# thedonutfactory/rs-tfhe

Hardware: AMD Instinct MI355X
Metric: gate-bootstraps/sec (hom_nand, SECURITY_128_BIT) (higher is better)
Workload: dtype f64

## Files before the change

rs-tfhe_amd/csrc/key_switch_mfma.hpp:

```cpp
#pragma once
#include <hip/hip_runtime.h>
#include <stdint.h>

#include <type_traits>

namespace tfhe {

constexpr int kKmWaves = 4;
constexpr int kKmFrags = 1;
constexpr int kKmRows = 32 * kKmFrags * kKmWaves;
constexpr int kKmSlots = 4;
constexpr int kKmAhead = kKmSlots - 1;
constexpr int kKmAbBytes = 32 * kKmFrags * 16 * 4;
constexpr int kKmAbQ = kKmAbBytes / 256;
constexpr int kKmColBlocks = 2;
constexpr int kKmMaxTiles = 12 / kKmFrags;

__host__ __device__ constexpr int ks_mfma_tpw(int nt) { return (nt + kKmWaves - 1) / kKmWaves; }
__host__ __device__ constexpr int ks_mfma_slot_bytes(int nt) { return ks_mfma_tpw(nt) * kKmWaves * 1024; }
__host__ __device__ constexpr size_t ks_mfma_lds_bytes(int nt) {
  return (size_t)kKmSlots * ks_mfma_slot_bytes(nt) + (size_t)kKmWaves * 2 * kKmAbBytes + (size_t)kKmWaves * 256;
}
__host__ __device__ __forceinline__ int ks_mfma_total_tiles(int n) { return (n + 1 + 31) / 32; }
__host__ __device__ __forceinline__ int ks_mfma_tiles(int n) { return (ks_mfma_total_tiles(n) + kKmColBlocks - 1) / kKmColBlocks; }
__host__ __device__ __forceinline__ int ks_mfma_block_tiles(int n, int cb) {
  const int tiles = ks_mfma_total_tiles(n);
  return tiles / kKmColBlocks + (cb < tiles % kKmColBlocks ? 1 : 0);
}
__host__ __device__ __forceinline__ int ks_mfma_block_first(int n, int cb) {
  const int tiles = ks_mfma_total_tiles(n), base = tiles / kKmColBlocks, rem = tiles % kKmColBlocks;
  return cb * base + (cb < rem ? cb : rem);
}
__host__ __device__ __forceinline__ size_t ks_mfma_key_bytes(int n, int t) {
  return (size_t)4 * (64 * 2 * t) * ks_mfma_total_tiles(n) * 1024;
}
constexpr size_t kKmKeyTailPad = 64 * 1024;

__host__ __device__ __forceinline__ uint32_t ks_plane_byte(uint32_t w, int p) {
  uint32_t s = 0;
  for (int q = 0; q <= p; ++q) {
    s = w & 0xFFu;
    const uint32_t sext = (s & 0x80u) ? (s | 0xFFFFFF00u) : s;
    w = (w - sext) >> 8;
  }
  return s;
}

template <class Word>
__device__ __forceinline__ uint4 ks_plane_fragment(int p, Word word) {
  uint32_t o[4];
#pragma unroll
  for (int q = 0; q < 4; ++q) {
    uint32_t d = 0;
#pragma unroll
    for (int e = 0; e < 4; ++e) d |= ks_plane_byte(word(q, e), p) << (8 * e);
    o[q] = d;
  }
  return make_uint4(o[0], o[1], o[2], o[3]);
}

__global__ void k_ksk_planes(const uint32_t *__restrict__ eng, unsigned char *__restrict__ out, int n, int t,
                             size_t chunks) {
  const size_t idx = (size_t)blockIdx.x * blockDim.x + threadIdx.x;
  if (idx >= chunks) return;
  const int lane = (int)(idx & 63);
  size_t r = idx >> 6;
  const int S = 64 * 2 * t, tiles = ks_mfma_total_tiles(n);
  const size_t per_plane = (size_t)S * tiles;
  const int p = (int)(r / per_plane);
  r -= (size_t)p * per_plane;
  int cb = 0;
  while (cb + 1 < kKmColBlocks && r >= (size_t)S * ks_mfma_block_first(n, cb + 1)) ++cb;
  r -= (size_t)S * ks_mfma_block_first(n, cb);
  const int nt = ks_mfma_block_tiles(n, cb);
  const int s = (int)(r / (size_t)nt), c = (int)(r % (size_t)nt);
  const int col = (ks_mfma_block_first(n, cb) + c) * 32 + (lane & 31), kb = lane >> 5;
  const int blk = s / (2 * t), u = s % (2 * t), j = u >> 1, hh = u & 1;
  const int rw = (n + 1 + 3) & ~3;
  reinterpret_cast<uint4 *>(out)[idx] = ks_plane_fragment(p, [=](int cc, int k) {
    const int i = 16 * blk + 8 * hh + 4 * kb + cc;
    const size_t row = ((size_t)i * t + j) * 4 + k;
    return (col <= n && k != 0) ? eng[row * (size_t)rw + col] : 0u;
  });
}

using km_i32x4 = __attribute__((ext_vector_type(4))) int;
using km_i32x16 = __attribute__((ext_vector_type(16))) int;
using km_u32x4 = __attribute__((ext_vector_type(4))) unsigned int;

__device__ __forceinline__ void km_dma16(uint32_t voff, const void *sbase, uint32_t lds) {
  uint32_t keep;
  asm volatile(
      "s_mov_b32 %0, m0\n\t"
      "s_mov_b32 m0, %3\n\t"
      "s_nop 0\n\t"
      "global_load_lds_dwordx4 %1, %2\n\t"
      "s_mov_b32 m0, %0"
      : "=&s"(keep)
      : "v"(voff), "s"(sbase), "s"(lds)
      : "memory");
}
__device__ __forceinline__ void km_dma4(uint32_t voff, const void *sbase, uint32_t lds) {
  uint32_t keep;
  asm volatile(
      "s_mov_b32 %0, m0\n\t"
      "s_mov_b32 m0, %3\n\t"
      "s_nop 0\n\t"
      "global_load_lds_dword %1, %2\n\t"
      "s_mov_b32 m0, %0"
      : "=&s"(keep)
      : "v"(voff), "s"(sbase), "s"(lds)
      : "memory");
}

struct KmPos {
  int blk, u;
};

template <int NT>
__global__ __launch_bounds__(64 * kKmWaves, 2) void k_key_switch_mfma(const uint32_t *__restrict__ lv1,
                                                                       const unsigned char *__restrict__ ksk8,
                                                                       int n, int t, uint32_t *__restrict__ out,
                                                                       size_t count,
                                                                       unsigned long long *clk,
                                                                       int ksplit) {
  constexpr int N = 1024, D = kKmAhead, WAVES = kKmWaves, R = kKmFrags;
  constexpr int TPW = ks_mfma_tpw(NT), SLOT = ks_mfma_slot_bytes(NT), OPS = TPW + R;
  const unsigned long long clk0 = clk ? __builtin_amdgcn_s_memtime() : 0ull;
  const unsigned long long rtc0 = clk ? __builtin_amdgcn_s_memrealtime() : 0ull;
  extern __shared__ __attribute__((aligned(16))) unsigned char km_smem[];
  const int tid = threadIdx.x, lane = tid & 63;
  const int wave = __builtin_amdgcn_readfirstlane(tid >> 6);
  const uint32_t lds_base = (uint32_t)(size_t)(__attribute__((address_space(3))) unsigned char *)km_smem;
  const uint32_t off_ab = (uint32_t)(kKmSlots * SLOT) + (uint32_t)wave * 2u * kKmAbBytes;
  const uint32_t off_dump = (uint32_t)(kKmSlots * SLOT) + (uint32_t)(WAVES * 2 * kKmAbBytes) + (uint32_t)wave * 256u;
  const unsigned lin = blockIdx.x + gridDim.x * (blockIdx.y + gridDim.y * blockIdx.z);
  const unsigned combos = gridDim.y * gridDim.z, combo = lin % combos, rest = lin / combos;
  const int cb = (int)(combo % gridDim.y), plane = (int)(combo / gridDim.y);
  const unsigned n_rb = gridDim.x / (unsigned)ksplit;
  const int kchunk = (int)(rest / n_rb);
  const int blk0 = kchunk * (64 / ksplit);
  const size_t row0 = (size_t)(rest % n_rb) * kKmRows + (size_t)wave * (32 * R);
  const int nt_blk = ks_mfma_block_tiles(n, cb), tile0 = ks_mfma_block_first(n, cb);
  const bool full = nt_blk == NT;
  const int spb = 2 * t, S = 64 * spb;
  const uint32_t prec = 1u << (31 - 2 * t);
  const uint32_t v16 = (uint32_t)lane * 16u;
  const uint32_t v4 = (uint32_t)(((lane >> 4) * (N + 1) + (lane & 15)) * 4);
  const uint32_t *ab_row0 = lv1 + row0 * (size_t)(N + 1);

  const unsigned char *kplane = ksk8 + ((size_t)plane * ks_mfma_total_tiles(n) + (size_t)tile0) * S * 1024;
  uint32_t koff[TPW];
#pragma unroll
  for (int i = 0; i < TPW; ++i) {
    const int tile = wave + i * WAVES;
    koff[i] = (uint32_t)(tile < nt_blk ? tile : nt_blk - 1) * 1024u + v16;
  }
  const uint32_t kstride = (uint32_t)nt_blk * 1024u;
  const int steps = S / ksplit;
#pragma unroll
  for (int i = 0; i < TPW; ++i) koff[i] += (uint32_t)(blk0 * spb) * kstride;
  auto dma_key = [&](uint32_t slot) {
#pragma unroll
    for (int i = 0; i < TPW; ++i) {
      km_dma16(koff[i], kplane, slot + (uint32_t)(wave + i * WAVES) * 1024u);
      koff[i] += kstride;
    }
  };

  for (int q = 0; q < kKmAbQ; ++q) km_dma4(v4, ab_row0 + (size_t)(4 * q) * (N + 1) + 16 * blk0, lds_base + off_ab + (uint32_t)q * 256u);
  for (int d = 0; d < D; ++d) dma_key(lds_base + (uint32_t)d * SLOT);
  asm volatile("s_waitcnt vmcnt(0)" ::: "memory");
  __builtin_amdgcn_s_barrier();
  asm volatile("" ::: "memory");

  km_i32x16 acc[R][NT];
  const uint32_t a_lane = (uint32_t)((lane & 31) * 64 + (lane >> 5) * 16);
  auto read_a = [&](const KmPos &q, int f) -> km_u32x4 {
    const unsigned char *abuf = km_smem + off_ab + (uint32_t)(q.blk & 1) * kKmAbBytes + a_lane + (uint32_t)(q.u & 1) * 32u;
    return *reinterpret_cast<const km_u32x4 *>(abuf + f * (32 * 64));
  };
  auto build_a = [&](const KmPos &q, km_u32x4 w) -> km_i32x4 {
    const uint32_t sh = (uint32_t)(27 - 2 * (q.u >> 1));
    km_u32x4 a;
    a.x = 1u << (((w.x + prec) >> sh) & 0x18u);
    a.y = 1u << (((w.y + prec) >> sh) & 0x18u);
    a.z = 1u << (((w.z + prec) >> sh) & 0x18u);
    a.w = 1u << (((w.w + prec) >> sh) & 0x18u);
    return __builtin_bit_cast(km_i32x4, a);
  };
  auto make_a = [&](const KmPos &q, int f) -> km_i32x4 { return build_a(q, read_a(q, f)); };
  KmPos cur{blk0, 0};
  km_i32x4 A[R];
#pragma unroll
  for (int f = 0; f < R; ++f) A[f] = make_a(cur, f);
  constexpr int PRE = NT < 3 ? NT : 3;
  constexpr int H = NT / 2;
  km_i32x4 Bpre[PRE];
#pragma unroll
  for (int c = 0; c < PRE; ++c) Bpre[c] = *reinterpret_cast<const km_i32x4 *>(km_smem + v16 + c * 1024);
#pragma unroll
  for (int f = 0; f < R; ++f)
#pragma unroll
    for (int c = 0; c < NT; ++c) acc[f][c] = km_i32x16{0, 0, 0, 0, 0, 0, 0, 0, 0, 0, 0, 0, 0, 0, 0, 0};
  auto run = [&](auto full_c) {
    constexpr bool FULL = decltype(full_c)::value;
#pragma unroll 1
    for (int g = 0; g < steps; ++g) {
      const unsigned char *slot = km_smem + (uint32_t)(g % kKmSlots) * SLOT + v16;
      const unsigned char *slot_next = km_smem + (uint32_t)((g + 1) % kKmSlots) * SLOT + v16;
      km_i32x4 B[NT];
#pragma unroll
      for (int c = 0; c < PRE; ++c) B[c] = Bpre[c];
#pragma unroll
      for (int c = 0; c < H; ++c) {
        if (c + PRE < NT) B[c + PRE] = *reinterpret_cast<const km_i32x4 *>(slot + (c + PRE) * 1024);
#pragma unroll
        for (int f = 0; f < R; ++f) acc[f][c] = __builtin_amdgcn_mfma_i32_32x32x32_i8(A[f], B[c], acc[f][c], 0, 0, 0);
      }
      __builtin_amdgcn_sched_barrier(0);
      asm volatile("s_waitcnt vmcnt(%0)" ::"n"((D - 2) * OPS) : "memory");
      __builtin_amdgcn_s_barrier();
      asm volatile("" ::: "memory");
      const uint32_t dslot = lds_base + (uint32_t)((g + D) % kKmSlots) * SLOT;
      const int nblk = (cur.blk + 1) & 63;
      const uint32_t nbuf = lds_base + off_ab + (uint32_t)((cur.blk + 1) & 1) * kKmAbBytes;
      const int u_now = cur.u;
      constexpr int PIECES = TPW + R + 2;
      km_i32x4 A_next[R];
      km_u32x4 Aw[R];
      auto piece = [&](int it) {
        if (it == 0) {
          if (++cur.u == spb) {
            cur.u = 0;
            cur.blk = (cur.blk + 1) & 63;
          }
#pragma unroll
          for (int f = 0; f < R; ++f) Aw[f] = read_a(cur, f);
#pragma unroll
          for (int c = 0; c < PRE; ++c) Bpre[c] = *reinterpret_cast<const km_i32x4 *>(slot_next + c * 1024);
        } else if (it == PIECES - 2) {
#pragma unroll
          for (int f = 0; f < R; ++f) A_next[f] = build_a(cur, Aw[f]);
        } else {
          const int d = it - 1 - (it > PIECES - 2 ? 1 : 0);
          if (d < TPW) {
            km_dma16(koff[d], kplane, dslot + (uint32_t)(wave + d * WAVES) * 1024u);
            koff[d] += kstride;
          } else {
            const int q0 = R * u_now + (d - TPW);
            const uint32_t *s0 = ab_row0 + (size_t)(4 * (q0 & (kKmAbQ - 1))) * (N + 1) + 16 * nblk;
            km_dma4(v4, s0, q0 < kKmAbQ ? nbuf + (uint32_t)q0 * 256u : lds_base + off_dump);
          }
        }
      };
#pragma unroll
      for (int c = H; c < NT; ++c) {
        if (c + PRE < NT) B[c + PRE] = *reinterpret_cast<const km_i32x4 *>(slot + (c + PRE) * 1024);
        if (c < NT - 1 || FULL) {
#pragma unroll
          for (int f = 0; f < R; ++f) acc[f][c] = __builtin_amdgcn_mfma_i32_32x32x32_i8(A[f], B[c], acc[f][c], 0, 0, 0);
        }
        __builtin_amdgcn_sched_barrier(0);
        if (c - H < PIECES) piece(c - H);
        __builtin_amdgcn_sched_barrier(0);
      }
#pragma unroll
      for (int it = NT - H; it < PIECES; ++it) piece(it);
#pragma unroll
      for (int f = 0; f < R; ++f) A[f] = A_next[f];
    }
  };
  if (full)
    run(std::true_type{});
  else
    run(std::false_type{});
  {
    const int sh8 = 8 * plane;
    const int row_lim = (int)(count > row0 ? (count - row0 < 32 * R ? count - row0 : 32 * R) : 0) - 4 * (lane >> 5);
    const int col_lane = tile0 * 32 + (lane & 31);
    const uint32_t lane_off = (uint32_t)((4 * (lane >> 5)) * (n + 1) + col_lane) * 4u;
    unsigned char *obase = reinterpret_cast<unsigned char *>(out + row0 * (size_t)(n + 1));
    const uint32_t row_bytes = (uint32_t)(n + 1) * 4u;
#pragma unroll
    for (int f = 0; f < R; ++f)
#pragma unroll
      for (int c = 0; c < NT; ++c) {
        const bool col_ok = col_lane + 32 * c <= n && c < nt_blk;
        const bool is_body = col_lane + 32 * c == n && plane == 0 && kchunk == 0;
#pragma unroll
        for (int e = 0; e < 16; ++e) {
          const int er = 32 * f + (e & 3) + 8 * (e >> 2);
          if (col_ok && er < row_lim) {
            uint32_t v = 0u - ((uint32_t)acc[f][c][e] << sh8);
            if (is_body) v += lv1[(row0 + (size_t)(er + 4 * (lane >> 5))) * (size_t)(N + 1) + N];
            unsigned char *uni = obase + (size_t)((uint32_t)er * row_bytes + (uint32_t)(c * 128));
            if (v) atomicAdd(reinterpret_cast<uint32_t *>(uni + lane_off), v);
          }
        }
      }
  }
  asm volatile("s_waitcnt vmcnt(0)" ::: "memory");
  if (clk && tid == 0) {
    atomicAdd(&clk[0], __builtin_amdgcn_s_memtime() - clk0);
    atomicAdd(&clk[1], __builtin_amdgcn_s_memrealtime() - rtc0);
  }
}

}
```

Before: 197,900.

## Use sparse SMFMAC i8 instructions for key-switch one-hot digit matmul

```diff
diff --git a/rs-tfhe_amd/csrc/key_switch_mfma.hpp b/rs-tfhe_amd/csrc/key_switch_mfma.hpp
--- a/rs-tfhe_amd/csrc/key_switch_mfma.hpp
+++ b/rs-tfhe_amd/csrc/key_switch_mfma.hpp
@@ -73,20 +73,28 @@
   while (cb + 1 < kKmColBlocks && r >= (size_t)S * ks_mfma_block_first(n, cb + 1)) ++cb;
   r -= (size_t)S * ks_mfma_block_first(n, cb);
   const int nt = ks_mfma_block_tiles(n, cb);
-  const int s = (int)(r / (size_t)nt), c = (int)(r % (size_t)nt);
-  const int col = (ks_mfma_block_first(n, cb) + c) * 32 + (lane & 31), kb = lane >> 5;
-  const int blk = s / (2 * t), u = s % (2 * t), j = u >> 1, hh = u & 1;
+  const int s = (int)(r / (size_t)(2 * nt)), c = (int)(r % (size_t)(2 * nt)) >> 1, q = (int)(r & 1);
+  const int col = (ks_mfma_block_first(n, cb) + c) * 32 + (lane & 31), h = lane >> 5;
+  const int blk = s / t, j = s % t;
   const int rw = (n + 1 + 3) & ~3;
   reinterpret_cast<uint4 *>(out)[idx] = ks_plane_fragment(p, [=](int cc, int k) {
-    const int i = 16 * blk + 8 * hh + 4 * kb + cc;
+    const int i = 16 * blk + 8 * h + 4 * q + cc;
     const size_t row = ((size_t)i * t + j) * 4 + k;
     return (col <= n && k != 0) ? eng[row * (size_t)rw + col] : 0u;
   });
 }
 
 using km_i32x4 = __attribute__((ext_vector_type(4))) int;
+using km_i32x8 = __attribute__((ext_vector_type(8))) int;
 using km_i32x16 = __attribute__((ext_vector_type(16))) int;
 using km_u32x4 = __attribute__((ext_vector_type(4))) unsigned int;
+
+constexpr int kKmSparseA = 0x00010001;
+__device__ __forceinline__ uint32_t km_sparse_idx(km_u32x4 lo, km_u32x4 hi, uint32_t prec, uint32_t sh) {
+  auto dg = [&](uint32_t w) { return ((w + prec) >> sh) & 3u; };
+  return dg(lo.x) | (dg(lo.y) << 4) | (dg(lo.z) << 8) | (dg(lo.w) << 12) | (dg(hi.x) << 16) | (dg(hi.y) << 20) |
+         (dg(hi.z) << 24) | (dg(hi.w) << 28);
+}
 
 __device__ __forceinline__ void km_dma16(uint32_t voff, const void *sbase, uint32_t lds) {
   uint32_t keep;
@@ -149,104 +157,116 @@
   const uint32_t v4 = (uint32_t)(((lane >> 4) * (N + 1) + (lane & 15)) * 4);
   const uint32_t *ab_row0 = lv1 + row0 * (size_t)(N + 1);
 
-  const unsigned char *kplane = ksk8 + ((size_t)plane * ks_mfma_total_tiles(n) + (size_t)tile0) * S * 1024;
-  uint32_t koff[TPW];
-#pragma unroll
-  for (int i = 0; i < TPW; ++i) {
-    const int tile = wave + i * WAVES;
-    koff[i] = (uint32_t)(tile < nt_blk ? tile : nt_blk - 1) * 1024u + v16;
-  }
-  const uint32_t kstride = (uint32_t)nt_blk * 1024u;
+  constexpr int T0 = (NT + 1) / 2, T1 = NT - T0;
+  static_assert(kKmSlots == 4 && D == 3, "unit g + D is the other half of a K-step: the ring arithmetic below");
+  static_assert(2 * T0 <= TPW * WAVES, "a unit's pieces fit the slot");
+  const uint32_t kstride = (uint32_t)nt_blk * 2048u;
+  const unsigned char *kwalk = ksk8 + ((size_t)plane * ks_mfma_total_tiles(n) + (size_t)tile0) * S * 1024 +
+                                (size_t)(blk0 * t) * kstride;
+  uint32_t spoff[2][TPW];
+#pragma unroll
+  for (int hf = 0; hf < 2; ++hf) {
+    const int up = hf ? 2 * (nt_blk - T0) : 2 * T0;
+#pragma unroll
+    for (int i = 0; i < TPW; ++i) {
+      const int pc = wave + i * WAVES, last = up > 0 ? up - 1 : 0;
+      spoff[hf][i] = (uint32_t)(hf * T0 * 2048) + (uint32_t)(pc < last ? pc : last) * 1024u;
+    }
+  }
   const int steps = S / ksplit;
-#pragma unroll
-  for (int i = 0; i < TPW; ++i) koff[i] += (uint32_t)(blk0 * spb) * kstride;
-  auto dma_key = [&](uint32_t slot) {
-#pragma unroll
-    for (int i = 0; i < TPW; ++i) {
-      km_dma16(koff[i], kplane, slot + (uint32_t)(wave + i * WAVES) * 1024u);
-      koff[i] += kstride;
-    }
+  auto dma_key = [&](int ks, int half, uint32_t slot) {
+    const unsigned char *src = kwalk + (size_t)ks * kstride;
+#pragma unroll
+    for (int i = 0; i < TPW; ++i) km_dma16(v16, src + spoff[half][i], slot + (uint32_t)(wave + i * WAVES) * 1024u);
   };
 
   for (int q = 0; q < kKmAbQ; ++q) km_dma4(v4, ab_row0 + (size_t)(4 * q) * (N + 1) + 16 * blk0, lds_base + off_ab + (uint32_t)q * 256u);
-  for (int d = 0; d < D; ++d) dma_key(lds_base + (uint32_t)d * SLOT);
+#pragma unroll
+  for (int d = 0; d < D; ++d) dma_key(d >> 1, d & 1, lds_base + (uint32_t)d * SLOT);
   asm volatile("s_waitcnt vmcnt(0)" ::: "memory");
   __builtin_amdgcn_s_barrier();
   asm volatile("" ::: "memory");
 
   km_i32x16 acc[R][NT];
   const uint32_t a_lane = (uint32_t)((lane & 31) * 64 + (lane >> 5) * 16);
-  auto read_a = [&](const KmPos &q, int f) -> km_u32x4 {
-    const unsigned char *abuf = km_smem + off_ab + (uint32_t)(q.blk & 1) * kKmAbBytes + a_lane + (uint32_t)(q.u & 1) * 32u;
+  auto read_a = [&](const KmPos &q, int f, int hi) -> km_u32x4 {
+    const unsigned char *abuf = km_smem + off_ab + (uint32_t)(q.blk & 1) * kKmAbBytes + a_lane + (uint32_t)hi * 32u;
     return *reinterpret_cast<const km_u32x4 *>(abuf + f * (32 * 64));
   };
-  auto build_a = [&](const KmPos &q, km_u32x4 w) -> km_i32x4 {
-    const uint32_t sh = (uint32_t)(27 - 2 * (q.u >> 1));
-    km_u32x4 a;
-    a.x = 1u << (((w.x + prec) >> sh) & 0x18u);
-    a.y = 1u << (((w.y + prec) >> sh) & 0x18u);
-    a.z = 1u << (((w.z + prec) >> sh) & 0x18u);
-    a.w = 1u << (((w.w + prec) >> sh) & 0x18u);
-    return __builtin_bit_cast(km_i32x4, a);
-  };
-  auto make_a = [&](const KmPos &q, int f) -> km_i32x4 { return build_a(q, read_a(q, f)); };
+  auto build_idx = [&](const KmPos &q, km_u32x4 lo, km_u32x4 hi) -> int {
+    return (int)km_sparse_idx(lo, hi, prec, (uint32_t)(30 - 2 * (q.u >> 1)));
+  };
+  auto read_b = [&](const unsigned char *slot, int c) -> km_i32x8 {
+    const km_i32x4 lo = *reinterpret_cast<const km_i32x4 *>(slot + c * 2048);
+    const km_i32x4 hi = *reinterpret_cast<const km_i32x4 *>(slot + c * 2048 + 1024);
+    return __builtin_shufflevector(lo, hi, 0, 1, 2, 3, 4, 5, 6, 7);
+  };
+  const km_i32x4 A1 = {kKmSparseA, kKmSparseA, kKmSparseA, kKmSparseA};
   KmPos cur{blk0, 0};
-  km_i32x4 A[R];
-#pragma unroll
-  for (int f = 0; f < R; ++f) A[f] = make_a(cur, f);
-  constexpr int PRE = NT < 3 ? NT : 3;
-  constexpr int H = NT / 2;
-  km_i32x4 Bpre[PRE];
-#pragma unroll
-  for (int c = 0; c < PRE; ++c) Bpre[c] = *reinterpret_cast<const km_i32x4 *>(km_smem + v16 + c * 1024);
+  int idx[R];
+#pragma unroll
+  for (int f = 0; f < R; ++f) idx[f] = build_idx(cur, read_a(cur, f, 0), read_a(cur, f, 1));
+  constexpr int PRE = R * NT * 16 > 176 ? 2 : 3;
+  km_i32x8 Bpre[PRE];
+#pragma unroll
+  for (int c = 0; c < (T0 < PRE ? T0 : PRE); ++c) Bpre[c] = read_b(km_smem + v16, c);
 #pragma unroll
   for (int f = 0; f < R; ++f)
 #pragma unroll
     for (int c = 0; c < NT; ++c) acc[f][c] = km_i32x16{0, 0, 0, 0, 0, 0, 0, 0, 0, 0, 0, 0, 0, 0, 0, 0};
-  auto run = [&](auto full_c) {
+  auto unit = [&](auto hf_c, auto full_c, int G) __attribute__((always_inline)) {
+    constexpr int HF = decltype(hf_c)::value;
     constexpr bool FULL = decltype(full_c)::value;
-#pragma unroll 1
-    for (int g = 0; g < steps; ++g) {
-      const unsigned char *slot = km_smem + (uint32_t)(g % kKmSlots) * SLOT + v16;
-      const unsigned char *slot_next = km_smem + (uint32_t)((g + 1) % kKmSlots) * SLOT + v16;
-      km_i32x4 B[NT];
-#pragma unroll
-      for (int c = 0; c < PRE; ++c) B[c] = Bpre[c];
+    constexpr int C0 = HF ? T0 : 0, TU = HF ? T1 : T0, TN = HF ? T0 : T1;
+    constexpr int PU = TU < PRE ? TU : PRE, PN = TN < PRE ? TN : PRE;
+    constexpr int H = TU > 1 ? 1 : 0;
+    {
+      const uint32_t sl = (uint32_t)(2 * (G & 1) + HF);
+      const unsigned char *slot = km_smem + sl * SLOT + v16;
+      const unsigned char *slot_next = km_smem + ((sl + 1u) & 3u) * SLOT + v16;
+      km_i32x8 B[TU > 0 ? TU : 1];
+#pragma unroll
+      for (int c = 0; c < PU; ++c) B[c] = Bpre[c];
 #pragma unroll
       for (int c = 0; c < H; ++c) {
-        if (c + PRE < NT) B[c + PRE] = *reinterpret_cast<const km_i32x4 *>(slot + (c + PRE) * 1024);
-#pragma unroll
-        for (int f = 0; f < R; ++f) acc[f][c] = __builtin_amdgcn_mfma_i32_32x32x32_i8(A[f], B[c], acc[f][c], 0, 0, 0);
+        if (c + PU < TU) B[c + PU] = read_b(slot, c + PU);
+#pragma unroll
+        for (int f = 0; f < R; ++f)
+          acc[f][C0 + c] = __builtin_amdgcn_smfmac_i32_32x32x64_i8(A1, B[c], acc[f][C0 + c], idx[f], 0, 0);
       }
       __builtin_amdgcn_sched_barrier(0);
       asm volatile("s_waitcnt vmcnt(%0)" ::"n"((D - 2) * OPS) : "memory");
       __builtin_amdgcn_s_barrier();
       asm volatile("" ::: "memory");
-      const uint32_t dslot = lds_base + (uint32_t)((g + D) % kKmSlots) * SLOT;
+      const uint32_t dslot = lds_base + ((sl + (uint32_t)D) & 3u) * SLOT;
       const int nblk = (cur.blk + 1) & 63;
       const uint32_t nbuf = lds_base + off_ab + (uint32_t)((cur.blk + 1) & 1) * kKmAbBytes;
       const int u_now = cur.u;
       constexpr int PIECES = TPW + R + 2;
-      km_i32x4 A_next[R];
-      km_u32x4 Aw[R];
+      const unsigned char *dsrc = kwalk + (size_t)(G + 1 + HF) * kstride;
+      int idx_next[R];
+      km_u32x4 Aw[R][2];
       auto piece = [&](int it) {
         if (it == 0) {
           if (++cur.u == spb) {
             cur.u = 0;
             cur.blk = (cur.blk + 1) & 63;
           }
-#pragma unroll
-          for (int f = 0; f < R; ++f) Aw[f] = read_a(cur, f);
-#pragma unroll
-          for (int c = 0; c < PRE; ++c) Bpre[c] = *reinterpret_cast<const km_i32x4 *>(slot_next + c * 1024);
+          if constexpr (HF == 1) {
+#pragma unroll
+            for (int f = 0; f < R; ++f) Aw[f][0] = read_a(cur, f, 0), Aw[f][1] = read_a(cur, f, 1);
+          }
+#pragma unroll
+          for (int c = 0; c < PN; ++c) Bpre[c] = read_b(slot_next, c);
         } else if (it == PIECES - 2) {
-#pragma unroll
-          for (int f = 0; f < R; ++f) A_next[f] = build_a(cur, Aw[f]);
+          if constexpr (HF == 1) {
+#pragma unroll
+            for (int f = 0; f < R; ++f) idx_next[f] = build_idx(cur, Aw[f][0], Aw[f][1]);
+          }
         } else {
           const int d = it - 1 - (it > PIECES - 2 ? 1 : 0);
           if (d < TPW) {
-            km_dma16(koff[d], kplane, dslot + (uint32_t)(wave + d * WAVES) * 1024u);
-            koff[d] += kstride;
+            km_dma16(v16, dsrc + spoff[HF ^ 1][d], dslot + (uint32_t)(wave + d * WAVES) * 1024u);
           } else {
             const int q0 = R * u_now + (d - TPW);
             const uint32_t *s0 = ab_row0 + (size_t)(4 * (q0 & (kKmAbQ - 1))) * (N + 1) + 16 * nblk;
@@ -255,20 +275,30 @@
         }
       };
 #pragma unroll
-      for (int c = H; c < NT; ++c) {
-        if (c + PRE < NT) B[c + PRE] = *reinterpret_cast<const km_i32x4 *>(slot + (c + PRE) * 1024);
-        if (c < NT - 1 || FULL) {
-#pragma unroll
-          for (int f = 0; f < R; ++f) acc[f][c] = __builtin_amdgcn_mfma_i32_32x32x32_i8(A[f], B[c], acc[f][c], 0, 0, 0);
+      for (int c = H; c < TU; ++c) {
+        if (c + PU < TU) B[c + PU] = read_b(slot, c + PU);
+        if (HF == 0 || c < TU - 1 || FULL) {
+#pragma unroll
+          for (int f = 0; f < R; ++f)
+            acc[f][C0 + c] = __builtin_amdgcn_smfmac_i32_32x32x64_i8(A1, B[c], acc[f][C0 + c], idx[f], 0, 0);
         }
         __builtin_amdgcn_sched_barrier(0);
         if (c - H < PIECES) piece(c - H);
         __builtin_amdgcn_sched_barrier(0);
       }
 #pragma unroll
-      for (int it = NT - H; it < PIECES; ++it) piece(it);
-#pragma unroll
-      for (int f = 0; f < R; ++f) A[f] = A_next[f];
+      for (int it = TU - H; it < PIECES; ++it) piece(it);
+      if constexpr (HF == 1) {
+#pragma unroll
+        for (int f = 0; f < R; ++f) idx[f] = idx_next[f];
+      }
+    }
+  };
+  auto run = [&](auto full_c) {
+#pragma unroll 1
+    for (int G = 0; G < steps / 2; ++G) {
+      unit(std::integral_constant<int, 0>{}, full_c, G);
+      unit(std::integral_constant<int, 1>{}, full_c, G);
     }
   };
   if (full)
```

New measurement: 197,400. About the same (-0.3%).
